# tnestmeyer/reflectance-filtering

Measured on AMD Instinct MI355X. Metric: megapixels/sec joint-bilateral sigma_c=20 sigma_s=22 @1080p, higher is better.
Workload: dtype f32

## Files before the change

### include/reflectance_filtering_debug.h

```cpp
#ifndef REFLECTANCE_FILTERING_DEBUG_H
#define REFLECTANCE_FILTERING_DEBUG_H

#ifdef __cplusplus
extern "C" {
#endif

int rf_debug_option(const char *name, int value);

int rf_debug_clock_probe(unsigned long long *out2, int micros, void *stream);

const char *rf_debug_build_info(void);

int rf_debug_jbf_points_plan(int n_params, const double *sigma_space, int d, int joint_cn, int flags,
                             int total_points, int *out, int max_chunks);

int rf_debug_jbf_ragged_plan(int n, const int *heights, const int *widths, int joint_cn, int src_cn,
                             int d, double sigma_color, double sigma_space, int flags, int *out,
                             int cap);

int rf_debug_jbf_ragged_slab_plan(int n, const int *heights, const int *widths, int joint_cn,
                                  int src_cn, int d, double sigma_color, double sigma_space, int flags,
                                  int *out, int cap);

int rf_debug_jbf_two_wg_plan(int n, int h, int w, int joint_cn, int src_cn, int d, double sigma_color,
                             double sigma_space, int flags, int *out);

int rf_debug_jbf_two_wg_calls(void);

int rf_debug_jbf_tile_flags(void *stream, unsigned char *out, int cap);

int rf_debug_colorize_ragged_plan(int n, const int *heights, const int *widths, int *out, int cap);

int rf_debug_gf_ragged_plan(int n, const int *heights, const int *widths, int guide_cn, int src_cn,
                            int radius, int flags, int *out, int cap);

int rf_debug_gf_launch_chunk(int chunk, int h, int w, int src_cn, int float_kernels);

int rf_debug_png_plan(int n, const int *heights, const int *widths, int cn_in, int flags, int *out,
                      int cap);

#ifdef __cplusplus
}
#endif
#endif
```

### reflectance_filtering_amd/_ffi.py

```python
import ctypes
import os
import threading

_HERE = os.path.dirname(os.path.abspath(__file__))
LIB_PATH = os.path.join(_HERE, "librf_hip.so")

RF_OK, RF_E_BADARG, RF_E_UNSUPPORTED, RF_E_WORKSPACE, RF_E_HIP = 0, -1, -2, -3, -4
BORDER_CONSTANT, BORDER_REPLICATE, BORDER_REFLECT, BORDER_WRAP, BORDER_REFLECT_101 = range(5)
BORDER_DEFAULT = BORDER_REFLECT_101
JBF_TRUE_DIVISION = 1
JBF_FORCE_GENERIC = 2
JBF_GREY_AS_BGR = 4
GF_GREY_AS_BGR = 1
PNG_GREY_AS_RGB = 1
PNG_FLAG_GREY, PNG_FLAG_BAD_FILTER = 1, 2
CNN_NPARAMS = 4513
CNN_NPACKED = 4673
CNN_NCHW_RGB, CNN_NHWC_BGR = 0, 1
CNN_LAYOUTS = {"nchw_rgb": CNN_NCHW_RGB, "nhwc_bgr": CNN_NHWC_BGR}

EXPORTS = ("rf_version", "rf_last_error", "rf_shutdown", "rf_jbf_u8", "rf_gf_workspace_bytes",
           "rf_gf_u8", "rf_gf_ex_u8", "rf_cnn_reflectance_u8", "rf_cnn_pack_weights",
           "rf_cnn_reflectance_packed_u8", "rf_colorize_workspace_bytes",
           "rf_colorize_srgb_u8", "rf_whdr_f32", "rf_jbf_f32_workspace_bytes", "rf_jbf_f32",
           "rf_gf_f32_workspace_bytes", "rf_gf_f32", "rf_jbf_points_workspace_bytes",
           "rf_jbf_points_u8", "rf_jbf_points_ragged_workspace_bytes", "rf_jbf_points_ragged_u8",
           "rf_whdr_points_u8", "rf_jbf_ragged_workspace_bytes", "rf_jbf_ragged_u8",
           "rf_colorize_ragged_workspace_bytes", "rf_colorize_ragged_srgb_u8",
           "rf_gf_ragged_workspace_bytes", "rf_gf_ragged_u8", "rf_png_stream_bound",
           "rf_png_workspace_bytes", "rf_png_deflate_ragged_u8",
           "rf_png_unfilter_workspace_bytes", "rf_png_unfilter_ragged_u8",
           "rf_colorize_ragged_r8_srgb_u8", "rf_cnn_reflectance_f32",
           "rf_cnn_reflectance_packed_f32", "rf_jbf_release_scratch")

DEBUG_EXPORTS = ("rf_debug_option", "rf_debug_clock_probe", "rf_debug_build_info",
                 "rf_debug_jbf_points_plan", "rf_debug_jbf_ragged_plan",
                 "rf_debug_jbf_ragged_slab_plan", "rf_debug_jbf_two_wg_plan",
                 "rf_debug_jbf_two_wg_calls", "rf_debug_jbf_tile_flags",
                 "rf_debug_colorize_ragged_plan",
                 "rf_debug_gf_ragged_plan", "rf_debug_gf_launch_chunk", "rf_debug_png_plan")
RESULT_CHANGING_OPTIONS = ("jbf_stage_only", "gf_exp_skip")

_lib = None
_lock = threading.Lock()


class RFError(RuntimeError):
    """A librf_hip.so entry point returned a negative code."""


def load_library():
    global _lib
    with _lock:
        if _lib is not None:
            return _lib
        import torch
        if not os.path.exists(LIB_PATH):
            raise RFError("%s not found: build it with `python -c 'import __graft_entry__ as g; "
                          "g.build()'` or `make -C reflectance_filtering_amd/csrc` "
                          "(there is no CPU fallback)" % LIB_PATH)
        lib = ctypes.CDLL(LIB_PATH)
        vp, ci, cd, sz = ctypes.c_void_p, ctypes.c_int, ctypes.c_double, ctypes.c_size_t
        lib.rf_version.argtypes = []
        lib.rf_version.restype = ci
        lib.rf_last_error.argtypes = []
        lib.rf_last_error.restype = ctypes.c_char_p
        lib.rf_shutdown.argtypes = []
        lib.rf_shutdown.restype = ci
        lib.rf_jbf_release_scratch.argtypes = []
        lib.rf_jbf_release_scratch.restype = ci
        lib.rf_jbf_u8.argtypes = [vp, vp, vp, ci, ci, ci, ci, ci, ci, cd, cd, ci, ci, vp]
        lib.rf_jbf_u8.restype = ci
        lib.rf_gf_workspace_bytes.argtypes = [ci, ci, ci, ci, ci, ci]
        lib.rf_gf_workspace_bytes.restype = sz
        lib.rf_gf_u8.argtypes = [vp, vp, vp, ci, ci, ci, ci, ci, ci, cd, ci, vp, sz, vp]
        lib.rf_gf_u8.restype = ci
        lib.rf_gf_ex_u8.argtypes = [vp, vp, vp, ci, ci, ci, ci, ci, ci, cd, ci, ci, vp, sz, vp]
        lib.rf_gf_ex_u8.restype = ci
        lib.rf_gf_ragged_workspace_bytes.argtypes = [ci, vp, vp, ci, ci, ci, ci]
        lib.rf_gf_ragged_workspace_bytes.restype = sz
        lib.rf_gf_ragged_u8.argtypes = [vp, vp, vp, ci, vp, vp, ci, ci, ci, cd, ci, ci, vp, sz, vp]
        lib.rf_gf_ragged_u8.restype = ci
        lib.rf_cnn_reflectance_u8.argtypes = [vp, vp, vp, ci, ci, ci, vp, vp, vp]
        lib.rf_cnn_reflectance_u8.restype = ci
        lib.rf_cnn_pack_weights.argtypes = [vp, vp, vp]
        lib.rf_cnn_pack_weights.restype = ci
        lib.rf_cnn_reflectance_packed_u8.argtypes = [vp, vp, vp, ci, ci, ci, vp, vp, vp]
        lib.rf_cnn_reflectance_packed_u8.restype = ci
        lib.rf_cnn_reflectance_f32.argtypes = [vp, vp, vp, ci, ci, ci, ci, vp, vp]
        lib.rf_cnn_reflectance_f32.restype = ci
# ... 14 lines not shown
        lib.rf_jbf_f32_workspace_bytes.restype = sz
        lib.rf_jbf_f32.argtypes = [vp, vp, vp, ci, ci, ci, ci, ci, ci, cd, cd, ci, vp, sz, vp]
        lib.rf_jbf_f32.restype = ci
        lib.rf_gf_f32_workspace_bytes.argtypes = [ci, ci, ci, ci, ci, ci]
        lib.rf_gf_f32_workspace_bytes.restype = sz
        lib.rf_gf_f32.argtypes = [vp, vp, vp, ci, ci, ci, ci, ci, ci, cd, ci, vp, sz, vp]
        lib.rf_gf_f32.restype = ci
        lib.rf_whdr_f32.argtypes = [vp, ci, ci, ci, ci, vp, vp, vp, cd, vp, vp]
        lib.rf_whdr_f32.restype = ci
        lib.rf_jbf_points_workspace_bytes.argtypes = [ci, vp, ci, ci, ci]
        lib.rf_jbf_points_workspace_bytes.restype = sz
        lib.rf_jbf_points_u8.argtypes = [vp, vp, ci, ci, ci, ci, ci, vp, vp, ci, ci, vp, vp, ci, ci,
                                         ci, vp, vp, sz, vp]
        lib.rf_jbf_points_u8.restype = ci
        lib.rf_jbf_points_ragged_workspace_bytes.argtypes = [ci, ci, vp, ci, ci, ci]
        lib.rf_jbf_points_ragged_workspace_bytes.restype = sz
        lib.rf_jbf_points_ragged_u8.argtypes = [vp, vp, ci, vp, vp, ci, ci, vp, vp, ci, ci, vp, vp, ci,
                                                ci, ci, vp, vp, sz, vp]
        lib.rf_jbf_points_ragged_u8.restype = ci
        lib.rf_jbf_ragged_workspace_bytes.argtypes = [ci, vp, vp, ci, ci, ci, cd, ci]
        lib.rf_jbf_ragged_workspace_bytes.restype = sz
        lib.rf_jbf_ragged_u8.argtypes = [vp, vp, vp, ci, vp, vp, ci, ci, ci, cd, cd, ci, ci, vp, sz,
                                         vp]
        lib.rf_jbf_ragged_u8.restype = ci
        lib.rf_whdr_points_u8.argtypes = [vp, ci, ctypes.c_longlong, ci, ci, vp, vp, vp, vp, cd, vp,
                                          vp]
        lib.rf_whdr_points_u8.restype = ci
        lib.rf_png_stream_bound.argtypes = [ci, vp, vp, ci, ci]
        lib.rf_png_stream_bound.restype = sz
        lib.rf_png_workspace_bytes.argtypes = [ci, vp, vp, ci, ci]
        lib.rf_png_workspace_bytes.restype = sz
        lib.rf_png_deflate_ragged_u8.argtypes = [vp, ci, vp, vp, ci, ci, vp, sz, vp, vp, sz, vp]
        lib.rf_png_deflate_ragged_u8.restype = ci
        lib.rf_png_unfilter_workspace_bytes.argtypes = [ci, vp, vp, vp]
        lib.rf_png_unfilter_workspace_bytes.restype = sz
        lib.rf_png_unfilter_ragged_u8.argtypes = [vp, vp, ci, vp, vp, vp, vp, vp, vp, vp, sz, vp]
        lib.rf_png_unfilter_ragged_u8.restype = ci
        lib.rf_debug_png_plan.argtypes = [ci, vp, vp, ci, ci, vp, ci]
        lib.rf_debug_png_plan.restype = ci
        lib.rf_debug_option.argtypes = [ctypes.c_char_p, ci]
        lib.rf_debug_option.restype = ci
        lib.rf_debug_clock_probe.argtypes = [vp, ci, vp]
        lib.rf_debug_clock_probe.restype = ci
        lib.rf_debug_build_info.argtypes = []
        lib.rf_debug_build_info.restype = ctypes.c_char_p
        lib.rf_debug_jbf_points_plan.argtypes = [ci, vp, ci, ci, ci, ci, vp, ci]
        lib.rf_debug_jbf_points_plan.restype = ci
        lib.rf_debug_jbf_ragged_plan.argtypes = [ci, vp, vp, ci, ci, ci, cd, cd, ci, vp, ci]
        lib.rf_debug_jbf_ragged_plan.restype = ci
        lib.rf_debug_jbf_ragged_slab_plan.argtypes = [ci, vp, vp, ci, ci, ci, cd, cd, ci, vp, ci]
        lib.rf_debug_jbf_ragged_slab_plan.restype = ci
        lib.rf_debug_jbf_two_wg_plan.argtypes = [ci, ci, ci, ci, ci, ci, cd, cd, ci, vp]
        lib.rf_debug_jbf_two_wg_plan.restype = ci
        lib.rf_debug_jbf_two_wg_calls.argtypes = []
        lib.rf_debug_jbf_two_wg_calls.restype = ci
        lib.rf_debug_jbf_tile_flags.argtypes = [vp, vp, ci]
        lib.rf_debug_jbf_tile_flags.restype = ci
        lib.rf_debug_colorize_ragged_plan.argtypes = [ci, vp, vp, vp, ci]
        lib.rf_debug_colorize_ragged_plan.restype = ci
        lib.rf_debug_gf_ragged_plan.argtypes = [ci, vp, vp, ci, ci, ci, ci, vp, ci]
        lib.rf_debug_gf_ragged_plan.restype = ci
        lib.rf_debug_gf_launch_chunk.argtypes = [ci, ci, ci, ci, ci]
        lib.rf_debug_gf_launch_chunk.restype = ci
        import sys
        for item in filter(None, os.environ.get("RF_DEBUG_OPTIONS", "").split(",")):
            name, _, value = item.partition("=")
            name = name.strip()
            try:
                number = int(value or 1)
            except ValueError:
                raise RFError("RF_DEBUG_OPTIONS: %r is not an integer (option %r)" % (value, name))
            if lib.rf_debug_option(name.encode(), number) < 0:
                raise RFError("RF_DEBUG_OPTIONS: unknown debug option %r" % name)
            if name in RESULT_CHANGING_OPTIONS and number:
                sys.stderr.write("reflectance_filtering_amd: WARNING: RF_DEBUG_OPTIONS sets %s=%d, a "
                                 "TIMING-ONLY switch - results of this process are WRONG\n"
                                 % (name, number))
            else:
                sys.stderr.write("reflectance_filtering_amd: RF_DEBUG_OPTIONS sets %s=%d\n"
                                 % (name, number))
        _lib = lib
        return lib


class debug_options:

    def __init__(self, **opts):
        self.opts = opts
        self.prev = {}

    def __enter__(self):
        lib = load_library()
        for name, value in self.opts.items():
            old = lib.rf_debug_option(name.encode(), int(value))
            if old < 0:
                raise ValueError("unknown debug option %r" % name)
            self.prev[name] = old
        return self

    def __exit__(self, *exc):
        lib = load_library()
        for name, old in self.prev.items():
            lib.rf_debug_option(name.encode(), old)
        return False


# ... 24 lines not shown
    import numpy as np
    lib = load_library()
    sizes = np.asarray(sizes, dtype=np.int64).reshape(-1, 2)
    hs = np.ascontiguousarray(sizes[:, 0], dtype=np.int32)
    ws = np.ascontiguousarray(sizes[:, 1], dtype=np.int32)
    out = np.zeros((4, 4), dtype=np.int32)
    rc = lib.rf_debug_jbf_ragged_plan(sizes.shape[0], hs.ctypes.data, ws.ctypes.data, int(joint_cn),
                                      int(src_cn), int(d), float(sigma_color), float(sigma_space),
                                      int(flags), out.ctypes.data, 4)
    if rc == -1:
        if sizes.shape[0] == 0 or lib.rf_jbf_ragged_workspace_bytes(
                sizes.shape[0], hs.ctypes.data, ws.ctypes.data, int(joint_cn), int(src_cn), int(d),
                float(sigma_space), int(flags)) > 0:
            return None
        lib.rf_debug_jbf_ragged_plan(sizes.shape[0], hs.ctypes.data, ws.ctypes.data, int(joint_cn),
                                     int(src_cn), int(d), float(sigma_color), float(sigma_space),
                                     int(flags), out.ctypes.data, 4)
    if rc < 0:
        check(rc, "rf_debug_jbf_ragged_plan")
    return [tuple(int(v) for v in row) for row in out[:rc]]


def jbf_ragged_slab_plan(sizes, joint_cn, src_cn, d, sigma_color, sigma_space, flags=0):
    import numpy as np
    lib = load_library()
    sizes = np.asarray(sizes, dtype=np.int64).reshape(-1, 2)
    hs = np.ascontiguousarray(sizes[:, 0], dtype=np.int32)
    ws = np.ascontiguousarray(sizes[:, 1], dtype=np.int32)
    out = np.zeros(7, dtype=np.int32)
    args = (sizes.shape[0], hs.ctypes.data, ws.ctypes.data, int(joint_cn), int(src_cn), int(d),
            float(sigma_color), float(sigma_space), int(flags), out.ctypes.data, 1)
    rc = lib.rf_debug_jbf_ragged_slab_plan(*args)
    if rc == -1:
        if sizes.shape[0] == 0 or lib.rf_jbf_ragged_workspace_bytes(*(args[:6] + (args[7], args[8]))) > 0:
            return None
        lib.rf_debug_jbf_ragged_slab_plan(*args)
    if rc < 0:
        check(rc, "rf_debug_jbf_ragged_slab_plan")
    return tuple(int(v) for v in out)


def jbf_two_wg_plan(n, h, w, joint_cn, src_cn, d, sigma_color, sigma_space, flags=0):
    import numpy as np
    lib = load_library()
    out = np.zeros(4, dtype=np.int32)
    rc = lib.rf_debug_jbf_two_wg_plan(int(n), int(h), int(w), int(joint_cn), int(src_cn), int(d),
                                      float(sigma_color), float(sigma_space), int(flags),
                                      out.ctypes.data)
    if rc < 0:
        check(rc, "rf_debug_jbf_two_wg_plan")
    return tuple(int(v) for v in out[1:]) if rc == 1 else None


def jbf_tile_flags(stream, tiles):
    import numpy as np
    lib = load_library()
    out = np.zeros(int(tiles), dtype=np.uint8)
    rc = lib.rf_debug_jbf_tile_flags(stream, out.ctypes.data, int(tiles))
    if rc < 0:
        check(rc, "rf_debug_jbf_tile_flags")
    if rc != int(tiles):
        raise RFError("rf_debug_jbf_tile_flags: %d bytes where %d tiles were asked for" % (rc, tiles))
    return out


def colorize_ragged_plan(sizes):
    import numpy as np
    lib = load_library()
    sizes = np.asarray(sizes, dtype=np.int64).reshape(-1, 2)
    n = sizes.shape[0]
    hs = np.ascontiguousarray(sizes[:, 0], dtype=np.int32)
    ws = np.ascontiguousarray(sizes[:, 1], dtype=np.int32)
    out = np.zeros(n + 2, dtype=np.int32)
    rc = lib.rf_debug_colorize_ragged_plan(n, hs.ctypes.data, ws.ctypes.data, out.ctypes.data, n + 2)
    if rc < 0:
        check(rc, "rf_debug_colorize_ragged_plan")
    return int(out[0]), int(out[1]), [int(v) for v in out[2:]]


def gf_ragged_plan(sizes, guide_cn, src_cn, radius, flags=0):
    import numpy as np
    lib = load_library()
    sizes = np.asarray(sizes, dtype=np.int64).reshape(-1, 2)
    hs = np.ascontiguousarray(sizes[:, 0], dtype=np.int32)
    ws = np.ascontiguousarray(sizes[:, 1], dtype=np.int32)
    out = np.zeros(6, dtype=np.int32)
    rc = lib.rf_debug_gf_ragged_plan(sizes.shape[0], hs.ctypes.data, ws.ctypes.data, int(guide_cn),
                                     int(src_cn), int(radius), int(flags), out.ctypes.data, 6)
    if rc < 0:
        check(rc, "rf_debug_gf_ragged_plan")
    if rc == 0:
        return None
    return dict(zip(("launches", "stage1", "rowstate", "colwalk", "hl", "out_w"),
                    (int(v) for v in out)))


def png_plan(sizes, cn_in=1, flags=0):
    import numpy as np
    lib = load_library()
    sizes = np.asarray(sizes, dtype=np.int64).reshape(-1, 2)
    n = sizes.shape[0]
    hs = np.ascontiguousarray(sizes[:, 0], dtype=np.int32)
    ws = np.ascontiguousarray(sizes[:, 1], dtype=np.int32)
    out = np.zeros(n + 2, dtype=np.int32)
    rc = lib.rf_debug_png_plan(n, hs.ctypes.data, ws.ctypes.data, int(cn_in), int(flags),
                               out.ctypes.data, n + 2)
# ... 16 lines not shown
```

### reflectance_filtering_amd/csrc/rf_api.hip

```cpp
#include "rf_common.hpp"

#include <atomic>
#include <cstring>

#include "reflectance_filtering_debug.h"

namespace rf {

void jbf_shutdown();
void jbf_scratch_release();
void cnn_shutdown();
void gf_shutdown();

char *last_error_buf()
{
    static thread_local char buf[512] = "";
    return buf;
}

int fail(int code, const char *fmt, ...)
{
    va_list ap;
    va_start(ap, fmt);
    vsnprintf(last_error_buf(), 512, fmt, ap);
    va_end(ap);
    return code;
}

static std::atomic<int> g_debug[kDbgCount];

int debug_get(int id) { return g_debug[id].load(std::memory_order_relaxed); }

}

extern "C" int rf_debug_option(const char *name, int value)
{
    static const char *const names[] = {"gf_two_kernel",     "jbf_stage_only",
                                                      "jbf_compiler_loop", "jbf_tile64_only",
                                                      "jbf_tune",          "jbf_f32_untiled",
                                                      "cnn_lds_columns",   "gf_seg_rows",
                                                      "gf_one_stream",     "gf_force_two_streams",
                                                      "gf_guide_cache",    "gf_chained",        "gf_no_compact",
                                                      "gf_exp_skip",       "gf_stagger",        "gf_parts",
                                                      "gf_s1_cap",         "gf_s1_min_wgs",
                                                      "jbf_lookahead1",    "gf_s1_legacy_strips",
                                                      "gf_exact_all_flagged", "gf_cw_chan_run",   "gf_exact",
                                                      "jbf_no_msad",       "colorize_chunk_px",
                                                      "jbf_no_two_wg",     "jbf_vote_scan",
                                                      "jbf_no_dead_skip"};
    static_assert(sizeof(names) / sizeof(names[0]) == rf::kDbgCount, "one name per DebugOption");
    if (name)
        for (int i = 0; i < rf::kDbgCount; i++)
            if (std::strcmp(name, names[i]) == 0)
                return rf::g_debug[i].exchange(value < 0 ? 0 : value);
    return rf::fail(RF_E_BADARG, "rf_debug_option: unknown option '%s'", name ? name : "(null)");
}

__global__ void clock_probe_kernel(unsigned long long *out, unsigned long long ticks)
{
    if (threadIdx.x != 0)
        return;
    const unsigned long long r0 = __builtin_amdgcn_s_memrealtime();
    const unsigned long long c0 = __builtin_amdgcn_s_memtime();
    unsigned long long r1 = r0;
    while (r1 - r0 < ticks) {
        __builtin_amdgcn_s_sleep(64);
        r1 = __builtin_amdgcn_s_memrealtime();
    }
    const unsigned long long c1 = __builtin_amdgcn_s_memtime();
    r1 = __builtin_amdgcn_s_memrealtime();
    out[0] = c1 - c0;
    out[1] = r1 - r0;
}

extern "C" int rf_debug_clock_probe(unsigned long long *out2, int micros, void *stream)
{
    if (!out2 || micros < 1 || micros > 1000000)
        return rf::fail(RF_E_BADARG, "rf_debug_clock_probe: bad argument");
    hipLaunchKernelGGL(clock_probe_kernel, dim3(1), dim3(64), 0, (hipStream_t)stream, out2,
                       (unsigned long long)micros * 100ull);
    RF_HIP_CHECK(hipGetLastError());
    return RF_OK;
}

#ifdef RF_GF_DEV_ONLY
extern "C" int rf_version(void) { return RF_VERSION | 0x40000000; }
#else
extern "C" int rf_version(void) { return RF_VERSION; }
#endif

#ifndef RF_TOOLCHAIN
#define RF_TOOLCHAIN "unknown toolchain"
#endif
extern "C" const char *rf_debug_build_info(void) { return RF_TOOLCHAIN; }

extern "C" const char *rf_last_error(void) { return rf::last_error_buf(); }

extern "C" int rf_shutdown(void)
{
    rf::jbf_shutdown();
    rf::jbf_scratch_release();
    rf::cnn_shutdown();
// ... 4 lines not shown
```

### reflectance_filtering_amd/csrc/rf_common.hpp

```cpp
#pragma once
#include <hip/hip_runtime.h>

#include <cstdarg>
#include <cstdint>
#include <cstdio>

#include "reflectance_filtering.h"

namespace rf {

char *last_error_buf();
int fail(int code, const char *fmt, ...);

#define RF_HIP_CHECK(expr)                                                                   \
    do {                                                                                     \
        hipError_t _e = (expr);                                                              \
        if (_e != hipSuccess)                                                                \
            return ::rf::fail(RF_E_HIP, "%s failed: %s (%s:%d)", #expr, hipGetErrorString(_e), \
                              __FILE__, __LINE__);                                           \
    } while (0)

__host__ __device__ inline int border_interpolate(int p, int len, int border)
{
    if ((unsigned)p < (unsigned)len)
// ... 31 lines not shown
inline int ceil_div(int a, int b) { return (a + b - 1) / b; }

inline bool launch_fits(unsigned long long workgroups, unsigned threads)
{
    return workgroups <= 0x7fffffffull && workgroups * threads < (1ull << 32);
}
constexpr int kMaxGridYZ = 65535;

inline bool ranges_overlap(const void *a, size_t na, const void *b, size_t nb)
{
    const uintptr_t a0 = (uintptr_t)a, b0 = (uintptr_t)b;
    return a0 < b0 + nb && b0 < a0 + na;
}

inline bool stream_is_capturing(hipStream_t stream)
{
    hipStreamCaptureStatus cs = hipStreamCaptureStatusNone;
    if (hipStreamIsCapturing(stream, &cs) != hipSuccess) {
        (void)hipGetLastError();
        return false;
    }
    return cs != hipStreamCaptureStatusNone;
}

enum DebugOption {
    kDbgGfTwoKernel = 0,
    kDbgJbfStageOnly,
    kDbgJbfCompilerLoop,
    kDbgJbfTile64Only,
    kDbgJbfTune,
    kDbgJbfF32Untiled,
    kDbgCnnLdsColumns,
    kDbgGfSegRows,
    kDbgGfOneStream,
    kDbgGfForceTwoStreams,
    kDbgGfGuideCache,
    kDbgGfChained,
    kDbgGfNoCompact,
    kDbgGfExpSkip,
    kDbgGfStagger,
    kDbgGfParts,
    kDbgGfS1Cap,
    kDbgGfS1MinWgs,
    kDbgJbfLookahead1,
    kDbgGfS1LegacyStrips,
    kDbgGfExactAllFlagged,
    kDbgGfCwChanRun,
    kDbgGfExact,
    kDbgJbfNoMsad,
    kDbgColorizeChunkPx,
    kDbgJbfNoTwoWg,
    kDbgJbfVoteScan,
    kDbgJbfNoDeadSkip,
    kDbgCount
};
int debug_get(int id);

}
```

### reflectance_filtering_amd/csrc/rf_jbf.hip

```cpp
#include <algorithm>
#include <atomic>
#include <mutex>
#include <vector>

#include "rf_jbf_common.hpp"
#include "rf_jbf_tables.hpp"
#include "rf_jbf_taploops.hpp"

namespace rf {
namespace {

constexpr int kTileW = 64;
constexpr int kMaxLds = 160 * 1024;
constexpr int kTlw2 = 144;
constexpr int kJbfMaxTiledR4 = 468;
constexpr int kJbfStageOnly = 0x1000, kJbfCompilerLoop = 0x2000, kJbfTile64Only = 0x4000;
constexpr int kJbfLookahead1 = 0x8000;
constexpr int kJbfNoMsad = 0x10000;
constexpr int kJbfVoteOnly = 0x20000;
constexpr int kJbfNoDeadSkip = 0x40000;

int jbf_debug_flags()
{
    return (debug_get(kDbgJbfStageOnly) ? kJbfStageOnly : 0) |
           (debug_get(kDbgJbfCompilerLoop) ? kJbfCompilerLoop : 0) |
           (debug_get(kDbgJbfTile64Only) ? kJbfTile64Only : 0) |
           (debug_get(kDbgJbfLookahead1) ? kJbfLookahead1 : 0) |
           (debug_get(kDbgJbfNoMsad) ? kJbfNoMsad : 0) |
           (debug_get(kDbgJbfNoDeadSkip) ? kJbfNoDeadSkip : 0);
}

__device__ inline void load_packed4(const uint8_t *img, size_t pix, int cn, uint32_t (&out)[4])
{
    const uint8_t *p = img + pix * (cn < 0 ? 1 : cn);
    if (cn == 3) {
        uint32_t d0, d1, d2;
        __builtin_memcpy(&d0, p, 4);
        __builtin_memcpy(&d1, p + 4, 4);
        __builtin_memcpy(&d2, p + 8, 4);
        out[0] = d0 & 0x00ffffffu;
        out[1] = (d0 >> 24) | ((d1 & 0xffffu) << 8);
        out[2] = (d1 >> 16) | ((d2 & 0xffu) << 16);
        out[3] = d2 >> 8;
    } else {
        uint32_t d0;
        __builtin_memcpy(&d0, p, 4);
        const uint32_t rep = cn < 0 ? 0x010101u : 1u;
        out[0] = (d0 & 0xffu) * rep;
        out[1] = ((d0 >> 8) & 0xffu) * rep;
        out[2] = ((d0 >> 16) & 0xffu) * rep;
        out[3] = (d0 >> 24) * rep;
    }
}

__device__ inline void load_tile_quad(const uint8_t *joint, const uint8_t *src, size_t img, int gy,
                                      int x_first, int w, int jcn, int scn, int border,
                                      uint32_t (&jv)[4], uint32_t (&sv)[4])
{
    if (gy < 0) {
#pragma unroll
        for (int u = 0; u < 4; u++)
            jv[u] = sv[u] = 0u;
        return;
    }
    const size_t row = img + (size_t)gy * w;
    if (x_first >= 0 && x_first + 3 < w) {
        load_packed4(joint, row + x_first, jcn, jv);
        load_packed4(src, row + x_first, scn, sv);
        return;
    }
#pragma unroll
    for (int u = 0; u < 4; u++) {
        const int gx = border_interpolate(x_first + u, w, border);
        jv[u] = gx < 0 ? 0u : load_packed(joint, row + gx, jcn);
        sv[u] = gx < 0 ? 0u : load_packed(src, row + gx, scn);
    }
}

__device__ inline int xcd_contiguous_tile(int b, int nblocks)
{
    const int per = nblocks >> 3;
    return b < (per << 3) ? (b & 7) * per + (b >> 3) : b;
// ... 1053 lines not shown
    const int r4 = (radius + 3) & ~3;
    const int tx = tid % QW, ty = tid / QW;
    int grey_joint = 1;
    if (flags & kJbfVoteOnly) {
        int grey = 1;
        const int rows_all = 64 + 2 * radius;
        for (int item = tid; item < rows_all * Q4; item += NT) {
            const int ry = item / Q4, k = item - ry * Q4;
            const int gy = border_interpolate(tile_y0 - radius + ry, h, border);
            uint32_t jv[4], sv[4];
            load_tile_quad(joint, src, img, gy, tile_x0 - r4 + 4 * k, w, jcn, scn, border, jv, sv);
#pragma unroll
            for (int u = 0; u < 4; u++) {
                if (scn == 3)
                    grey &= (int)(((sv[u] ^ (sv[u] >> 8)) & 0xffffu) == 0u);
                if (jcn == 3)
                    grey_joint &= (int)(((jv[u] ^ (jv[u] >> 8)) & 0xffffu) == 0u);
            }
        }
        const int bits = block_all2(grey, grey_joint, flag_word);
        if (tid == 0)
            tile_flags[tile_id] = (uint8_t)(((bits & 1) ? 0 : 1) | (bits & 2));
        return;
    }
    if (tile_flags) {
        const int byte = __builtin_amdgcn_readfirstlane((int)tile_flags[tile_id]);
        if (byte & 1)
            return;
        grey_joint = (byte >> 1) & 1;
    }
    float *lut_g = reinterpret_cast<float *>(smem + kT64x2Lds - nz * GREP * 4);
    for (int i = tid; i < nz * GREP; i += NT)
        lut_g[i] = lut[i / GREP];
    const uint32_t lut_lane_addr = lds_addr(lut_g) + (uint32_t)(tid & (GREP - 1)) * 4u;
    const uint32_t tile_lane_addr = lds_addr(tile4) + (uint32_t)tx * 4u;
    const bool j1 = grey_joint != 0;
    const uint32_t j1_scale = (uint32_t)(jcn == 1 ? 1 : 3) * (GREP * 4u);
    uint32_t jc[kPix];
    float sum1[kPix][1], wsum[kPix];
    {
        uint32_t jv[4], sv[4];
        load_tile_quad(joint, src, img, border_interpolate(tile_y0 + ty, h, border), tile_x0 + 4 * tx, w, jcn,
                       scn, border, jv, sv);
#pragma unroll
        for (int p = 0; p < kPix; p++) {
            jc[p] = j1 ? (jv[p] & 0xffu) * j1_scale : jv[p] & 0x00ffffffu;
            sum1[p][0] = 0.f;
            wsum[p] = 0.f;
        }
    }
    const bool msad = !j1 && !(flags & kJbfNoMsad) && jbf_wave_takes_msad(jc);
    const bool live_wave =
        __builtin_amdgcn_readfirstlane(tile_y0 + (ty & ~3)) < h || (flags & kJbfNoDeadSkip) != 0;
    for (int i0 = -radius; i0 <= radius; i0 += slab_rows) {
        const int i1 = min(i0 + slab_rows - 1, radius);
        const int tlh = 64 + (i1 - i0);
        __syncthreads();
        for (int item = tid; item < tlh * Q4; item += NT) {
            const int ry = item / Q4, k = item - ry * Q4;
            const int gy = border_interpolate(tile_y0 + i0 + ry, h, border);
            uint32_t jv[4], sv[4];
            load_tile_quad(joint, src, img, gy, tile_x0 - r4 + 4 * k, w, jcn, scn, border, jv, sv);
#pragma unroll
            for (int u = 0; u < 4; u++) {
                const uint32_t jfield = j1 ? (jv[u] & 0xffu) * j1_scale : jv[u];
                tile4[ry * TLW + u * Q4 + k] = jfield | (sv[u] << 24);
            }
        }
        __syncthreads();
        if (!live_wave)
            continue;
        if (j1)
            jbf_tap_loop_grey4_la2<GREP, TLW, true, true>(lut_lane_addr, swsym, tile_lane_addr, jc, ty,
                                                          radius, r4, sw_len, hwtab, sum1, wsum, i0, i1, -i0);
        else if (msad)
            jbf_tap_loop_grey4_la2<GREP, TLW, false, true, true>(lut_lane_addr, swsym, tile_lane_addr, jc,
                                                                 ty, radius, r4, sw_len, hwtab, sum1, wsum,
                                                                 i0, i1, -i0);
        else
            jbf_tap_loop_grey4_la2<GREP, TLW, false, true>(lut_lane_addr, swsym, tile_lane_addr, jc, ty,
                                                           radius, r4, sw_len, hwtab, sum1, wsum, i0, i1,
                                                           -i0);
    }
    if (scn == 1)
        store_quad<1, 1>(dst, img, tile_y0 + ty, tile_x0 + 4 * tx, h, w, sum1, wsum, flags);
    else
        store_quad<1, 3>(dst, img, tile_y0 + ty, tile_x0 + 4 * tx, h, w, sum1, wsum, flags);
}

struct TileFlagBuf {
    int dev;
    hipStream_t stream;
    uint8_t *p;
    size_t bytes;
};
std::mutex g_tf_mu;
std::vector<TileFlagBuf> g_tf;
std::vector<uint8_t *> g_tf_retired;
constexpr size_t kTileFlagStreams = 16;
std::atomic<int> g_two_wg_calls{0};

size_t tile_flag_bytes(size_t tiles)
{
    size_t b = 4096;
    while (b < tiles)
        b <<= 1;
    return b;
}

int get_tile_flags(int dev, hipStream_t stream, size_t tiles, uint8_t **out)
{
    *out = nullptr;
    std::lock_guard<std::mutex> lock(g_tf_mu);
    size_t at = g_tf.size();
    for (size_t i = 0; i < g_tf.size(); i++)
        if (g_tf[i].dev == dev && g_tf[i].stream == stream)
            at = i;
    if (at < g_tf.size() && g_tf[at].bytes >= tiles) {
        *out = g_tf[at].p;
        return RF_OK;
    }
    hipStreamCaptureStatus st = hipStreamCaptureStatusNone;
    if (hipStreamIsCapturing(stream, &st) != hipSuccess || st != hipStreamCaptureStatusNone) {
        (void)hipGetLastError();
        return RF_OK;
    }
    if (at == g_tf.size() && g_tf.size() >= kTileFlagStreams)
        return RF_OK;
    uint8_t *p = nullptr;
    {
        CaptureRelax relax;
        RF_HIP_CHECK(hipMalloc(&p, tile_flag_bytes(tiles)));
    }
    if (at < g_tf.size()) {
        g_tf_retired.push_back(g_tf[at].p);
        g_tf.erase(g_tf.begin() + at);
    }
    g_tf.push_back(TileFlagBuf{dev, stream, p, tile_flag_bytes(tiles)});
    *out = p;
    return RF_OK;
}

bool two_wg_choose(const JbfTables &t, int nz, int src_cn, int flags, int *slab_rows)
{
    *slab_rows = 0;
    if (debug_get(kDbgJbfNoTwoWg) || debug_get(kDbgJbfTune) ||
        (flags & (RF_JBF_FORCE_GENERIC | kJbfStageOnly | kJbfCompilerLoop | kJbfLookahead1)))
        return false;
    Tile64Shape shape;
    if (t.r4 > 36 || !tile64_choose(t, nz, src_cn, flags, &shape) || shape.tlw != 144 || shape.grep != 32)
        return false;
    *slab_rows = tile64x2_slab_rows(nz, 32, 144);
    return *slab_rows >= 8;
}

int launch_tile64x2(const JbfTables &t, int nz, int slab_rows, const uint8_t *joint, const uint8_t *src,
                    uint8_t *dst, int n, int h, int w, int jcn, int scn, int border, int flags,
                    hipStream_t stream, int rows, int cols, uint8_t *tile_flags)
{
    const int tiles_x = ceil_div(cols, 64), tiles_y = ceil_div(rows, 64);
    const long long blocks = (long long)tiles_x * tiles_y * n;
    auto kern = jbf_tile64x2_kernel<32, 144>;
    RF_HIP_CHECK(hipFuncSetAttribute((const void *)kern, hipFuncAttributeMaxDynamicSharedMemorySize,
                                     kT64x2Lds));
    hipLaunchKernelGGL(kern, dim3((unsigned)blocks), dim3(1024), kT64x2Lds, stream, joint, src, dst, h, w,
                       jcn, scn, t.radius, border, t.d_lut, nz, t.d_hw, t.d_swsym, t.sw_len, tiles_x,
                       tiles_x * tiles_y, flags, slab_rows, tile_flags);
    return RF_OK;
}

template <int CREP>
int launch_tile64_flagged(const JbfTables &t, int nz, int crows, const uint8_t *joint, const uint8_t *src,
                          uint8_t *dst, int n, int h, int w, int jcn, int border, int flags,
                          hipStream_t stream, int rows, int cols, const uint8_t *tile_flags)
{
    const int tiles_x = ceil_div(cols, 64), tiles_y = ceil_div(rows, 64);
    const long long blocks = (long long)tiles_x * tiles_y * n;
    auto kern = jbf_tile64_kernel<3, 32, CREP, 144, 64, false, true>;
    RF_HIP_CHECK(hipFuncSetAttribute((const void *)kern, hipFuncAttributeMaxDynamicSharedMemorySize,
                                     kT64Lds));
    hipLaunchKernelGGL(kern, dim3((unsigned)blocks), dim3(1024), kT64Lds, stream, joint, src, dst, h, w,
                       jcn, t.radius, border, t.d_lut, nz, t.d_hw, t.d_swsym, t.sw_len, tiles_x,
                       tiles_x * tiles_y, flags, crows, 0, 0, tile_flags);
    return RF_OK;
}

int launch_two_wg(const JbfTables &t, int nz, const Tile64Shape &shape, int slab_rows,
                  const uint8_t *joint, const uint8_t *src, uint8_t *dst, int n, int h, int w, int jcn,
                  int scn, int border, int flags, hipStream_t stream, bool *done)
{
    *done = false;
    const Tile64Areas a = tile64_areas(t, nz, shape.grep, shape.crep, scn, flags, h, w);
    if (a.rows_main <= 0 || a.cols_main <= 0)
        return RF_OK;
    const long long blocks = (long long)ceil_div(a.cols_main, 64) * ceil_div(a.rows_main, 64) * n;
    if (!launch_fits(blocks, 1024))
        return fail(RF_E_UNSUPPORTED, "rf_jbf_u8: batch too large for one launch");
    uint8_t *tile_flags = nullptr;
    int rc = RF_OK;
    if (scn == 3 || jcn == 3) {
        if (int bad = get_tile_flags(t.device, stream, (size_t)blocks, &tile_flags))
            return bad;
        if (!tile_flags)
            return RF_OK;
        const int tiles_x = ceil_div(a.cols_main, 64), tiles_y = ceil_div(a.rows_main, 64);
        if (debug_get(kDbgJbfVoteScan) || !jbf_grey_map_serves(h, w, t.radius, border, tiles_x, tiles_y))
// ... 290 lines not shown
    const JbfTables t = jbf_host_tables(jbf_radius(d, jbf_sigma(sigma_space)),
                                        jbf_table_cn(joint_cn, flags), jbf_sigma(sigma_color),
                                        jbf_sigma(sigma_space), lut);
    RaggedPlan plan;
    plan_ragged(t, n, heights, widths, src_cn, flags | jbf_debug_flags(),
                debug_get(kDbgJbfTune) & 0xf, &plan);
    if (!plan.tiled)
        return -1;
    int launches = 0;
    for (int c = 0; c < kRaggedClasses; c++) {
        if (plan.recs[c].empty())
            continue;
        if (launches < cap) {
            out[4 * launches + 0] = kRaggedTh[c];
            out[4 * launches + 1] = 4096 / kRaggedTh[c];
            out[4 * launches + 2] = plan.shape.tlw == 144 ? kRaggedPitch144[c] : plan.shape.tlw;
            out[4 * launches + 3] = (int)std::min<size_t>(plan.recs[c].size(), 0x7fffffff);
        }
        launches++;
    }
    return launches;
}

extern "C" int rf_debug_jbf_ragged_slab_plan(int n, const int *heights, const int *widths,
                                             int joint_cn, int src_cn, int d, double sigma_color,
                                             double sigma_space, int flags, int *out, int cap)
{
    using namespace rf;
    const char *who = "rf_debug_jbf_ragged_slab_plan";
    size_t px, tiles;
    if (cap < 0 || (cap > 0 && !out))
        return fail(RF_E_BADARG, "%s: bad cap=%d", who, cap);
    if (int bad = ragged_check(who, n, heights, widths, joint_cn, src_cn, d, sigma_space,
                               RF_BORDER_DEFAULT, flags, &px, &tiles))
        return bad;
    std::vector<float> lut;
    const JbfTables t = jbf_host_tables(jbf_radius(d, jbf_sigma(sigma_space)),
                                        jbf_table_cn(joint_cn, flags), jbf_sigma(sigma_color),
                                        jbf_sigma(sigma_space), lut);
    RaggedPlan plan;
    plan_ragged(t, n, heights, widths, src_cn, flags | jbf_debug_flags(),
                debug_get(kDbgJbfTune) & 0xf, &plan);
    if (!plan.slab)
        return -1;
    if (cap > 0) {
        const SlabShape &s = plan.slab_shape;
        const int record[7] = {s.tlw, s.grep, s.crows_g, s.slab_g, s.crows_c, s.slab_c,
                               (int)std::min<size_t>(plan.recs[0].size(), 0x7fffffff)};
        std::copy(record, record + 7, out);
    }
    return 1;
}

extern "C" int rf_debug_jbf_two_wg_plan(int n, int h, int w, int joint_cn, int src_cn, int d,
                                        double sigma_color, double sigma_space, int flags, int *out)
{
    using namespace rf;
    const char *who = "rf_debug_jbf_two_wg_plan";
    size_t px, tiles;
    if (n < 1 || !out)
        return fail(RF_E_BADARG, "%s: bad n=%d or NULL out", who, n);
    if (int bad = ragged_check(who, 1, &h, &w, joint_cn, src_cn, d, sigma_space, RF_BORDER_DEFAULT, flags,
                               &px, &tiles))
        return bad;
    std::vector<float> lut;
    const JbfTables t = jbf_host_tables(jbf_radius(d, jbf_sigma(sigma_space)),
                                        jbf_table_cn(joint_cn, flags), jbf_sigma(sigma_color),
                                        jbf_sigma(sigma_space), lut);
    flags |= jbf_debug_flags();
    const int nz = t.lut_len < 256 * t.joint_cn ? t.lut_len - 1 : t.lut_len;
    out[0] = out[1] = out[2] = out[3] = 0;
    int slab_rows = 0;
    Tile64Shape shape;
    if (t.r4 > kJbfMaxTiledR4 || !two_wg_choose(t, nz, src_cn, flags, &slab_rows) ||
        !tile64_choose(t, nz, src_cn, flags, &shape))
        return 0;
    const Tile64Areas a = tile64_areas(t, nz, shape.grep, shape.crep, src_cn, flags, h, w);
    const long long blocks = (long long)ceil_div(a.cols_main, 64) * ceil_div(a.rows_main, 64) * n;
    if (a.rows_main <= 0 || a.cols_main <= 0 || !launch_fits(blocks, 1024))
        return 0;
    out[0] = 1;
    out[1] = 64 + slab_rows - 1;
    out[2] = (int)blocks;
    out[3] = src_cn == 3 || joint_cn == 3 ? (int)tile_flag_bytes((size_t)blocks) : 0;
    return 1;
}

extern "C" int rf_jbf_ragged_u8(const uint8_t *joint, const uint8_t *src, uint8_t *dst, int n,
                                const int *heights, const int *widths, int joint_cn, int src_cn,
                                int d, double sigma_color, double sigma_space, int border, int flags,
                                void *workspace, size_t workspace_bytes, void *stream_)
{
    using namespace rf;
    const char *who = "rf_jbf_ragged_u8";
    if (n == 0)
        return RF_OK;
    if (!joint || !src || !dst)
        return fail(RF_E_BADARG, "%s: NULL image pointer", who);
    size_t px, tiles;
    if (int bad = ragged_check(who, n, heights, widths, joint_cn, src_cn, d, sigma_space, border,
                               flags, &px, &tiles))
        return bad;
    if (ranges_overlap(dst, px * src_cn, joint, px * joint_cn) ||
        ranges_overlap(dst, px * src_cn, src, px * src_cn))
        return fail(RF_E_BADARG, "%s: dst must not overlap an input", who);
    if (!workspace || workspace_bytes < ragged_bytes(tiles) || ((uintptr_t)workspace & 15))
        return fail(RF_E_BADARG, "%s: workspace of %zu bytes, %zu needed (16-byte aligned)", who,
                    workspace ? workspace_bytes : (size_t)0, ragged_bytes(tiles));
    hipStream_t stream = (hipStream_t)stream_;
    if (stream_is_capturing(stream))
        return fail(RF_E_UNSUPPORTED, "%s: synchronises its stream and cannot be captured into a "
                                      "graph", who);
    const int user_flags = flags;
    flags |= jbf_debug_flags();
    const double sc = jbf_sigma(sigma_color), ss = jbf_sigma(sigma_space);
    const int radius = jbf_radius(d, ss);
    const int jcn_kernel = jbf_kernel_cn(joint_cn, flags);
    const int table_cn = jbf_table_cn(joint_cn, flags);
    const int tune = debug_get(kDbgJbfTune) & 0xf;
    RaggedPlan plan;
    JbfTables t;
    TablesHold hold{t};
    if (!(flags & RF_JBF_FORCE_GENERIC) && tune == 0 && ((radius + 3) & ~3) <= kJbfMaxTiledR4) {
        int rc = get_tables(radius, table_cn, sc, ss, stream, &t);
        if (rc != RF_OK)
            return rc;
        bool oob_ok = false;
        rc = lds_oob_reads_zero(t.device, &oob_ok);
        if (rc != RF_OK)
            return rc;
        if (oob_ok)
            plan_ragged(t, n, heights, widths, src_cn, flags, tune, &plan);
    }
    if (!plan.tiled && !plan.slab) {
        size_t first = 0;
        for (int i = 0; i < n; i++) {
            const int rc = rf_jbf_u8(joint + first * joint_cn, src + first * src_cn,
// ... 54 lines not shown
```

### reflectance_filtering_amd/csrc/rf_jbf_taploops.hpp

```cpp
#pragma once
#include <type_traits>

#include "rf_common.hpp"

namespace rf {
namespace {

constexpr int kPix = 4;

typedef uint32_t uint2v __attribute__((ext_vector_type(2)));
typedef float float4v __attribute__((ext_vector_type(4)));

#define RF_LDS_READ_B64(dst, addr, off) \
    asm volatile("ds_read_b64 %0, %1 offset:%2" : "=v"(dst) : "v"(addr), "n"(off))
#define RF_LDS_READ_B128(dst, addr, off) \
    asm volatile("ds_read_b128 %0, %1 offset:%2" : "=v"(dst) : "v"(addr), "n"(off))
#define RF_LDS_READ_B32(dst, addr) asm volatile("ds_read_b32 %0, %1" : "=v"(dst) : "v"(addr))
#define RF_LDS_READ_B32_OFF(dst, addr, off) \
    asm volatile("ds_read_b32 %0, %1 offset:%2" : "=v"(dst) : "v"(addr), "n"(off))
#define RF_LDS_READ_U16_OFF(dst, addr, off) \
    asm volatile("ds_read_u16 %0, %1 offset:%2" : "=v"(dst) : "v"(addr), "n"(off))

template <int NCH, int LUTREP, bool CLAMP, int TLW, int TB>
__device__ __forceinline__ void jbf_tap_loop(uint32_t lut_lane_addr, uint32_t sw_addr0,
// ... 344 lines not shown
                P1(1, gg[1], gg[0], ta, 0, 0)                                                       \
                RF_G4_PART2(tp[1], gg[0], )                                                         \
            }                                                                                       \
            {                                                                                       \
                P1(2, gg[0], gg[1], ta_next, 0, Q4 * 4)                                             \
                RF_G4_PART2(tp[0], gg[1], )                                                         \
            }                                                                                       \
            {                                                                                       \
                P1(3, gg[1], gg[0], ta_next, 0, 0)                                                  \
                RF_LOAD_WINDOW(wa_next)                                                             \
                RF_G4_PART2(tp[0], gg[0], RF_COMMA_W)                                               \
            }                                                                                       \
        }                                                                                           \
        ta = ta_next;                                                                               \
        wa_addr = wa_next;                                                                          \
        ngroups = ngroups_next;                                                                     \
    }
    if constexpr (J1) {
        RF_ROW_LOOP(RF_G4_PART1_J1)
    } else {
        RF_ROW_LOOP(RF_G4_PART1)
    }
#undef RF_ROW_LOOP
#undef RF_G4_PART1_J1
#undef RF_LOAD_WINDOW
#undef RF_COMMA_W
#undef RF_G4_PART1
#undef RF_G4_PART2
#undef RF_TEXEL_OFF4
#undef RF_TQ
#undef RF_G4_READ
#undef RF_G4_READ_0
#undef RF_G4_READ_1
#undef RF_G4_READ_2
#undef RF_G4_READ_3
#undef RF_G4_TNOUT
#undef RF_G4_TNOUT_0
#undef RF_G4_TNOUT_1
#undef RF_G4_TNOUT_2
#undef RF_G4_TNOUT_3
}

__device__ __forceinline__ bool jbf_wave_takes_msad(const uint32_t (&jc)[kPix], bool counts = true)
{
    uint32_t z = 0u;
#pragma unroll
    for (int p = 0; p < kPix; p++) {
        const uint32_t v = jc[p] | 0xff000000u;
        z |= (v - 0x01010101u) & ~v & 0x80808080u;
    }
    return __ballot(counts && z != 0u) == 0ull;
}

template <int LUTREP, int TLW, bool J1 = false, bool SLAB = false, bool MSAD = false>
__device__ __forceinline__ void jbf_tap_loop_grey4_la2(uint32_t lut_lane_addr,
                                                       const float *__restrict__ swsym,
                                                       uint32_t tile_lane_addr,
                                                       const uint32_t (&jc)[kPix], int ty, int radius,
                                                       int r4, int sw_len,
                                                       const int *__restrict__ hwtab,
                                                       float (&sum)[kPix][1], float (&wsum)[kPix],
                                                       int i_first = 0, int i_last = 0, int row_bias = 0)
{
    const int i_lo = SLAB ? i_first : -radius, i_hi = SLAB ? i_last : radius;
    const int bias = SLAB ? row_bias : radius;
    constexpr int Q4 = TLW / 4;
    constexpr int SHIFT = LUTREP == 32 ? 7 : LUTREP == 16 ? 6 : LUTREP == 8 ? 5 : 4;
    static_assert(LUTREP == 32 || LUTREP == 16 || LUTREP == 8 || LUTREP == 4, "LUT replicas");
    static_assert(Q4 + 2 <= 255, "ds_read2_b32 offsets are 8 bits (the largest one here: Q4 + 2)");
    static_assert(TLW % 4 == 0, "column-interleaved planes");
    static_assert(!(MSAD && J1), "the single-channel form has no masked SAD");
    [[maybe_unused]] uint32_t mask = 0x00ffffffu;
    if constexpr (!MSAD)
        asm volatile("" : "+v"(mask));

    const uint32_t lane_row0 = tile_lane_addr + (uint32_t)(ty * TLW * 4);
    auto row_addr = [&](int i, int hw, uint32_t &ta_out, uint32_t &tb_out, uint32_t &wa_out,
                        int &ngroups_out) {
        const int hws = (hw + 1) & ~1;
        const int ai = i < 0 ? -i : i;
        const int c0 = r4 - hws;
        const int quad = (i + bias) * TLW + (c0 >> 2);
        const int phase = (c0 >> 1) & 1;
        ta_out = lane_row0 + (uint32_t)((quad + (phase ? 2 * Q4 : 0)) * 4);
        tb_out = lane_row0 + (uint32_t)((quad + (phase ? 1 : 2 * Q4)) * 4);
        wa_out = (uint32_t)(ai * sw_len + (r4 + 8) + hws - 4);
        ngroups_out = (hws + hw + 4 + 3) >> 2;
    };

    uint2v tp[2];
    typedef float float8v __attribute__((ext_vector_type(8)));
    float8v w8a, w8b;
    float gg[4][kPix];
    float sv[4];
    uint32_t ta, tb, wa_addr;
    int ngroups;
    int odd = 0;
    if constexpr (SLAB) {
        int hw0;
        const int *hp0 = hwtab + (i_lo + radius);
        asm volatile("s_load_dword %0, %1, 0x0\n\ts_waitcnt lgkmcnt(0)" : "=s"(hw0) : "s"(hp0));
        hw0 = __builtin_amdgcn_readfirstlane(hw0);
        odd = hw0 & 1;
        row_addr(i_lo, hw0, ta, tb, wa_addr, ngroups);
    } else {
        row_addr(-radius, 0, ta, tb, wa_addr, ngroups);
    }
    int hw_ahead, hw_cur;
    {
        const int *hp = SLAB ? hwtab + ((i_lo + 1 < i_hi ? i_lo + 1 : i_hi) + radius) : hwtab + 1;
        asm volatile("s_load_dword %0, %1, 0x0" : "=s"(hw_ahead) : "s"(hp));
    }
    asm volatile("ds_read2_b32 %0, %2 offset1:%4\n\t"
                 "ds_read2_b32 %1, %3 offset1:%4"
                 : "=&v"(tp[0]), "=&v"(tp[1])
                 : "v"(ta), "v"(tb), "n"(Q4));
    {
        const float *wp = swsym + wa_addr;
        asm volatile("s_load_dwordx8 %0, %2, 0x0" : "=&s"(w8a), "=s"(w8b) : "s"(wp));
    }
    asm volatile("s_waitcnt lgkmcnt(0)" : "+v"(tp[0]), "+v"(tp[1]), "+s"(w8a), "+s"(w8b));
#pragma unroll
    for (int c = 0; c < 2; c++) {
        const uint32_t tx = c == 0 ? tp[0].x : tp[0].y;
        const uint32_t tj = MSAD ? tx : tx & mask;
#pragma unroll
        for (int p = 0; p < kPix; p++) {
            const uint32_t a =
                J1     ? (tj > jc[p] ? tj - jc[p] : jc[p] - tj) + lut_lane_addr
                : MSAD ? __builtin_amdgcn_msad_u8(tj, jc[p], 0u) * (LUTREP * 4u) + lut_lane_addr
                       : __builtin_amdgcn_sad_u8(tj, jc[p], 0u) * (LUTREP * 4u) + lut_lane_addr;
            asm volatile("ds_read_b32 %0, %1" : "=v"(gg[c][p]) : "v"(a));
        }
        sv[c] = (float)(tx >> 24);
    }
    asm volatile("s_waitcnt lgkmcnt(0)\n\t"
                 "s_mov_b32 %[hwc], %[hwa]"
                 : "+v"(gg[0][0]), "+v"(gg[0][1]), "+v"(gg[0][2]), "+v"(gg[0][3]), "+v"(gg[1][0]),
// ... 536 lines not shown
```

Measured before the change: 2662.

## Stage two-workgroup JBF tile rows in an LDS ring to avoid re-loading overlap

The slab loop of the two-workgroup 64-row tile kernel previously re-staged all 64+slab-1 rows into LDS for every slab, reloading the 63 overlapping rows each time. With a ring buffer, later slabs load only the new slab rows into the ring position, and the tap loop wraps its row addresses modulo the ring size. This cuts global loads and LDS writes per slab in exchange for an extra compare/select per row address. The ring is only used when the tile is at LDS address zero, and the two-WG path is now gated on the ring staging fewer rows. A debug option and a staged-rows plan query are added.

```diff
diff --git a/include/reflectance_filtering_debug.h b/include/reflectance_filtering_debug.h
--- a/include/reflectance_filtering_debug.h
+++ b/include/reflectance_filtering_debug.h
@@ -25,6 +25,9 @@
 int rf_debug_jbf_two_wg_plan(int n, int h, int w, int joint_cn, int src_cn, int d, double sigma_color,
                              double sigma_space, int flags, int *out);
 
+int rf_debug_jbf_two_wg_staged_rows(int n, int h, int w, int joint_cn, int src_cn, int d, double sigma_color,
+                                    double sigma_space, int flags, int *out);
+
 int rf_debug_jbf_two_wg_calls(void);
 
 int rf_debug_jbf_tile_flags(void *stream, unsigned char *out, int cap);
diff --git a/reflectance_filtering_amd/_ffi.py b/reflectance_filtering_amd/_ffi.py
--- a/reflectance_filtering_amd/_ffi.py
+++ b/reflectance_filtering_amd/_ffi.py
@@ -36,6 +36,7 @@
 DEBUG_EXPORTS = ("rf_debug_option", "rf_debug_clock_probe", "rf_debug_build_info",
                  "rf_debug_jbf_points_plan", "rf_debug_jbf_ragged_plan",
                  "rf_debug_jbf_ragged_slab_plan", "rf_debug_jbf_two_wg_plan",
+                 "rf_debug_jbf_two_wg_staged_rows",
                  "rf_debug_jbf_two_wg_calls", "rf_debug_jbf_tile_flags",
                  "rf_debug_colorize_ragged_plan",
                  "rf_debug_gf_ragged_plan", "rf_debug_gf_launch_chunk", "rf_debug_png_plan")
@@ -156,6 +157,8 @@
         lib.rf_debug_jbf_ragged_slab_plan.restype = ci
         lib.rf_debug_jbf_two_wg_plan.argtypes = [ci, ci, ci, ci, ci, ci, cd, cd, ci, vp]
         lib.rf_debug_jbf_two_wg_plan.restype = ci
+        lib.rf_debug_jbf_two_wg_staged_rows.argtypes = [ci, ci, ci, ci, ci, ci, cd, cd, ci, vp]
+        lib.rf_debug_jbf_two_wg_staged_rows.restype = ci
         lib.rf_debug_jbf_two_wg_calls.argtypes = []
         lib.rf_debug_jbf_two_wg_calls.restype = ci
         lib.rf_debug_jbf_tile_flags.argtypes = [vp, vp, ci]
@@ -286,6 +289,18 @@
     return tuple(int(v) for v in out[1:]) if rc == 1 else None
 
 
+def jbf_two_wg_staged_rows(n, h, w, joint_cn, src_cn, d, sigma_color, sigma_space, flags=0):
+    import numpy as np
+    lib = load_library()
+    out = np.zeros(3, dtype=np.int32)
+    rc = lib.rf_debug_jbf_two_wg_staged_rows(int(n), int(h), int(w), int(joint_cn), int(src_cn), int(d),
+                                             float(sigma_color), float(sigma_space), int(flags),
+                                             out.ctypes.data)
+    if rc < 0:
+        check(rc, "rf_debug_jbf_two_wg_staged_rows")
+    return tuple(int(v) for v in out) if rc == 1 else None
+
+
 def jbf_tile_flags(stream, tiles):
     import numpy as np
     lib = load_library()
diff --git a/reflectance_filtering_amd/csrc/rf_api.hip b/reflectance_filtering_amd/csrc/rf_api.hip
--- a/reflectance_filtering_amd/csrc/rf_api.hip
+++ b/reflectance_filtering_amd/csrc/rf_api.hip
@@ -47,7 +47,7 @@
                                                       "gf_exact_all_flagged", "gf_cw_chan_run",   "gf_exact",
                                                       "jbf_no_msad",       "colorize_chunk_px",
                                                       "jbf_no_two_wg",     "jbf_vote_scan",
-                                                      "jbf_no_dead_skip"};
+                                                      "jbf_no_dead_skip",  "jbf_no_ring"};
     static_assert(sizeof(names) / sizeof(names[0]) == rf::kDbgCount, "one name per DebugOption");
     if (name)
         for (int i = 0; i < rf::kDbgCount; i++)
diff --git a/reflectance_filtering_amd/csrc/rf_common.hpp b/reflectance_filtering_amd/csrc/rf_common.hpp
--- a/reflectance_filtering_amd/csrc/rf_common.hpp
+++ b/reflectance_filtering_amd/csrc/rf_common.hpp
@@ -107,6 +107,7 @@
     kDbgJbfNoTwoWg,
     kDbgJbfVoteScan,
     kDbgJbfNoDeadSkip,
+    kDbgJbfNoRing,
     kDbgCount
 };
 int debug_get(int id);
diff --git a/reflectance_filtering_amd/csrc/rf_jbf.hip b/reflectance_filtering_amd/csrc/rf_jbf.hip
--- a/reflectance_filtering_amd/csrc/rf_jbf.hip
+++ b/reflectance_filtering_amd/csrc/rf_jbf.hip
@@ -19,6 +19,7 @@
 constexpr int kJbfNoMsad = 0x10000;
 constexpr int kJbfVoteOnly = 0x20000;
 constexpr int kJbfNoDeadSkip = 0x40000;
+constexpr int kJbfNoRing = 0x80000;
 
 int jbf_debug_flags()
 {
@@ -27,7 +28,8 @@
            (debug_get(kDbgJbfTile64Only) ? kJbfTile64Only : 0) |
            (debug_get(kDbgJbfLookahead1) ? kJbfLookahead1 : 0) |
            (debug_get(kDbgJbfNoMsad) ? kJbfNoMsad : 0) |
-           (debug_get(kDbgJbfNoDeadSkip) ? kJbfNoDeadSkip : 0);
+           (debug_get(kDbgJbfNoDeadSkip) ? kJbfNoDeadSkip : 0) |
+           (debug_get(kDbgJbfNoRing) ? kJbfNoRing : 0);
 }
 
 __device__ inline void load_packed4(const uint8_t *img, size_t pix, int cn, uint32_t (&out)[4])
@@ -1187,35 +1189,43 @@
     const bool msad = !j1 && !(flags & kJbfNoMsad) && jbf_wave_takes_msad(jc);
     const bool live_wave =
         __builtin_amdgcn_readfirstlane(tile_y0 + (ty & ~3)) < h || (flags & kJbfNoDeadSkip) != 0;
+    const bool ring = (flags & kJbfNoRing) == 0 && lds_addr(tile4) == 0u;
+    const int ring_rows = 64 + slab_rows - 1;
     for (int i0 = -radius; i0 <= radius; i0 += slab_rows) {
         const int i1 = min(i0 + slab_rows - 1, radius);
-        const int tlh = 64 + (i1 - i0);
+        const bool add_only = ring && i0 > -radius;
+        const int nrows = add_only ? i1 - i0 + 1 : 64 + (i1 - i0);
+        const int t_first = add_only ? 63 : 0;
+        const int p_first = add_only ? i0 + radius + 63 - ring_rows : 0;
         __syncthreads();
-        for (int item = tid; item < tlh * Q4; item += NT) {
+        for (int item = tid; item < nrows * Q4; item += NT) {
             const int ry = item / Q4, k = item - ry * Q4;
-            const int gy = border_interpolate(tile_y0 + i0 + ry, h, border);
+            const int gy = border_interpolate(tile_y0 + i0 + t_first + ry, h, border);
             uint32_t jv[4], sv[4];
             load_tile_quad(joint, src, img, gy, tile_x0 - r4 + 4 * k, w, jcn, scn, border, jv, sv);
 #pragma unroll
             for (int u = 0; u < 4; u++) {
                 const uint32_t jfield = j1 ? (jv[u] & 0xffu) * j1_scale : jv[u];
-                tile4[ry * TLW + u * Q4 + k] = jfield | (sv[u] << 24);
+                tile4[(p_first + ry) * TLW + u * Q4 + k] = jfield | (sv[u] << 24);
             }
         }
         __syncthreads();
         if (!live_wave)
             continue;
+        constexpr bool kRing = true;
+        const int bias = ring ? radius : -i0;
         if (j1)
-            jbf_tap_loop_grey4_la2<GREP, TLW, true, true>(lut_lane_addr, swsym, tile_lane_addr, jc, ty,
-                                                          radius, r4, sw_len, hwtab, sum1, wsum, i0, i1, -i0);
+            jbf_tap_loop_grey4_la2<GREP, TLW, true, true, false, kRing>(lut_lane_addr, swsym, tile_lane_addr,
+                                                                        jc, ty, radius, r4, sw_len, hwtab, sum1,
+                                                                        wsum, i0, i1, bias, ring_rows);
         else if (msad)
-            jbf_tap_loop_grey4_la2<GREP, TLW, false, true, true>(lut_lane_addr, swsym, tile_lane_addr, jc,
-                                                                 ty, radius, r4, sw_len, hwtab, sum1, wsum,
-                                                                 i0, i1, -i0);
+            jbf_tap_loop_grey4_la2<GREP, TLW, false, true, true, kRing>(lut_lane_addr, swsym, tile_lane_addr,
+                                                                        jc, ty, radius, r4, sw_len, hwtab, sum1,
+                                                                        wsum, i0, i1, bias, ring_rows);
         else
-            jbf_tap_loop_grey4_la2<GREP, TLW, false, true>(lut_lane_addr, swsym, tile_lane_addr, jc, ty,
-                                                           radius, r4, sw_len, hwtab, sum1, wsum, i0, i1,
-                                                           -i0);
+            jbf_tap_loop_grey4_la2<GREP, TLW, false, true, false, kRing>(lut_lane_addr, swsym, tile_lane_addr,
+                                                                         jc, ty, radius, r4, sw_len, hwtab, sum1,
+                                                                         wsum, i0, i1, bias, ring_rows);
     }
     if (scn == 1)
         store_quad<1, 1>(dst, img, tile_y0 + ty, tile_x0 + 4 * tx, h, w, sum1, wsum, flags);
@@ -1286,7 +1296,15 @@
     if (t.r4 > 36 || !tile64_choose(t, nz, src_cn, flags, &shape) || shape.tlw != 144 || shape.grep != 32)
         return false;
     *slab_rows = tile64x2_slab_rows(nz, 32, 144);
-    return *slab_rows >= 8;
+    if (*slab_rows < 8)
+        return false;
+    return 63 + 2 * t.radius < 2 * (64 + *slab_rows - 1);
+}
+
+int two_wg_staged_rows(int radius, int slab_rows, bool ring)
+{
+    const int slabs = ceil_div(2 * radius + 1, slab_rows);
+    return ring ? 64 + 2 * radius : 63 * slabs + 2 * radius + 1;
 }
 
 int launch_tile64x2(const JbfTables &t, int nz, int slab_rows, const uint8_t *joint, const uint8_t *src,
@@ -1683,12 +1701,13 @@
     return 1;
 }
 
-extern "C" int rf_debug_jbf_two_wg_plan(int n, int h, int w, int joint_cn, int src_cn, int d,
-                                        double sigma_color, double sigma_space, int flags, int *out)
-{
-    using namespace rf;
-    const char *who = "rf_debug_jbf_two_wg_plan";
+namespace rf {
+namespace {
+int two_wg_plan(const char *who, int n, int h, int w, int joint_cn, int src_cn, int d, double sigma_color,
+                double sigma_space, int flags, int *out, int *slab_rows, int *radius)
+{
     size_t px, tiles;
+    *slab_rows = *radius = 0;
     if (n < 1 || !out)
         return fail(RF_E_BADARG, "%s: bad n=%d or NULL out", who, n);
     if (int bad = ragged_check(who, 1, &h, &w, joint_cn, src_cn, d, sigma_space, RF_BORDER_DEFAULT, flags,
@@ -1701,9 +1720,9 @@
     flags |= jbf_debug_flags();
     const int nz = t.lut_len < 256 * t.joint_cn ? t.lut_len - 1 : t.lut_len;
     out[0] = out[1] = out[2] = out[3] = 0;
-    int slab_rows = 0;
+    int rows = 0;
     Tile64Shape shape;
-    if (t.r4 > kJbfMaxTiledR4 || !two_wg_choose(t, nz, src_cn, flags, &slab_rows) ||
+    if (t.r4 > kJbfMaxTiledR4 || !two_wg_choose(t, nz, src_cn, flags, &rows) ||
         !tile64_choose(t, nz, src_cn, flags, &shape))
         return 0;
     const Tile64Areas a = tile64_areas(t, nz, shape.grep, shape.crep, src_cn, flags, h, w);
@@ -1711,9 +1730,39 @@
     if (a.rows_main <= 0 || a.cols_main <= 0 || !launch_fits(blocks, 1024))
         return 0;
     out[0] = 1;
-    out[1] = 64 + slab_rows - 1;
+    out[1] = 64 + rows - 1;
     out[2] = (int)blocks;
     out[3] = src_cn == 3 || joint_cn == 3 ? (int)tile_flag_bytes((size_t)blocks) : 0;
+    *slab_rows = rows;
+    *radius = t.radius;
+    return 1;
+}
+}
+}
+
+extern "C" int rf_debug_jbf_two_wg_plan(int n, int h, int w, int joint_cn, int src_cn, int d,
+                                        double sigma_color, double sigma_space, int flags, int *out)
+{
+    int slab_rows, radius;
+    return rf::two_wg_plan("rf_debug_jbf_two_wg_plan", n, h, w, joint_cn, src_cn, d, sigma_color, sigma_space,
+                           flags, out, &slab_rows, &radius);
+}
+
+extern "C" int rf_debug_jbf_two_wg_staged_rows(int n, int h, int w, int joint_cn, int src_cn, int d,
+                                               double sigma_color, double sigma_space, int flags, int *out)
+{
+    using namespace rf;
+    int plan[4], slab_rows, radius;
+    if (!out)
+        return fail(RF_E_BADARG, "rf_debug_jbf_two_wg_staged_rows: NULL out");
+    out[0] = out[1] = out[2] = 0;
+    const int rc = two_wg_plan("rf_debug_jbf_two_wg_staged_rows", n, h, w, joint_cn, src_cn, d, sigma_color,
+                               sigma_space, flags, plan, &slab_rows, &radius);
+    if (rc != 1)
+        return rc;
+    out[0] = slab_rows;
+    out[1] = ceil_div(2 * radius + 1, slab_rows);
+    out[2] = two_wg_staged_rows(radius, slab_rows, !debug_get(kDbgJbfNoRing));
     return 1;
 }
 
diff --git a/reflectance_filtering_amd/csrc/rf_jbf_taploops.hpp b/reflectance_filtering_amd/csrc/rf_jbf_taploops.hpp
--- a/reflectance_filtering_amd/csrc/rf_jbf_taploops.hpp
+++ b/reflectance_filtering_amd/csrc/rf_jbf_taploops.hpp
@@ -420,7 +420,7 @@
     return __ballot(counts && z != 0u) == 0ull;
 }
 
-template <int LUTREP, int TLW, bool J1 = false, bool SLAB = false, bool MSAD = false>
+template <int LUTREP, int TLW, bool J1 = false, bool SLAB = false, bool MSAD = false, bool RING = false>
 __device__ __forceinline__ void jbf_tap_loop_grey4_la2(uint32_t lut_lane_addr,
                                                        const float *__restrict__ swsym,
                                                        uint32_t tile_lane_addr,
@@ -428,8 +428,10 @@
                                                        int r4, int sw_len,
                                                        const int *__restrict__ hwtab,
                                                        float (&sum)[kPix][1], float (&wsum)[kPix],
-                                                       int i_first = 0, int i_last = 0, int row_bias = 0)
+                                                       int i_first = 0, int i_last = 0, int row_bias = 0,
+                                                       int ring_rows = 0)
 {
+    static_assert(!RING || SLAB, "a ring of rows is walked in slabs");
     const int i_lo = SLAB ? i_first : -radius, i_hi = SLAB ? i_last : radius;
     const int bias = SLAB ? row_bias : radius;
     constexpr int Q4 = TLW / 4;
@@ -450,8 +452,15 @@
         const int c0 = r4 - hws;
         const int quad = (i + bias) * TLW + (c0 >> 2);
         const int phase = (c0 >> 1) & 1;
-        ta_out = lane_row0 + (uint32_t)((quad + (phase ? 2 * Q4 : 0)) * 4);
-        tb_out = lane_row0 + (uint32_t)((quad + (phase ? 1 : 2 * Q4)) * 4);
+        if constexpr (RING) {
+            const uint32_t a = lane_row0 + (uint32_t)((quad + (phase ? 2 * Q4 : 0)) * 4);
+            const uint32_t wrapped = a - (uint32_t)(ring_rows * TLW * 4);
+            ta_out = a < wrapped ? a : wrapped;
+            tb_out = ta_out + (uint32_t)((phase ? 1 - 2 * Q4 : 2 * Q4) * 4);
+        } else {
+            ta_out = lane_row0 + (uint32_t)((quad + (phase ? 2 * Q4 : 0)) * 4);
+            tb_out = lane_row0 + (uint32_t)((quad + (phase ? 1 : 2 * Q4)) * 4);
+        }
         wa_out = (uint32_t)(ai * sw_len + (r4 + 8) + hws - 4);
         ngroups_out = (hws + hw + 4 + 3) >> 2;
     };
```

After: 2684, median of 6. Within noise of the previous version (+0.8%).
